# nibox/Pose-Estimation-with-Message-Passing-Networks

Hardware: AMD Instinct MI355X
Metric: images/sec (640px, HRNet-w48) + MPN edge-updates/sec at 1/2/4/8 MI355X (higher is better)
Workload: dtype f16x3; 1 GPU; c3: 8x17x640x640 heatmaps/GPU -> fully graph -> MPN TypeAware-attn T=3; images_per_gpu=8, global_batch=8, persons_per_image=9, nodes_per_gpu=1224, edges_per_gpu=186048, parallelism=image-sharded x1, batches_in_flight=2, detection_and_node_math=fp32

## Files before the change

### include/pemp.h

```cpp
#ifndef PEMP_H_
#define PEMP_H_

#include <stddef.h>
#include <stdint.h>

#ifdef __cplusplus
extern "C" {
#endif

#define PEMP_ABI_VERSION 24

enum {
  PEMP_OK = 0,
  PEMP_ERR_INVALID_ARG = -1,
  PEMP_ERR_HIP = -2,
  PEMP_ERR_WORKSPACE = -3,
  PEMP_ERR_UNSUPPORTED = -4,
};

int pemp_abi_version(void);
const char* pemp_last_error(void);
int pemp_device_check(void);

enum { PEMP_DETECT_NMS = 1, PEMP_DETECT_SELECT = 2, PEMP_DETECT_ALL = 3 };
// ... 215 lines not shown
                               const int32_t* n_det, int det_cap, const int64_t* node_off, int B,
                               float* edge_logits, float* node_logits, float* class_logits,
                               void* workspace, size_t workspace_bytes, void* stream);

enum {
  PEMP_STEP_DET = 0, PEMP_STEP_DSC, PEMP_STEP_NDET, PEMP_STEP_X, PEMP_STEP_JDET, PEMP_STEP_JSC, PEMP_STEP_BIDX,
  PEMP_STEP_JTAGS, PEMP_STEP_EIDX, PEMP_STEP_EATTR, PEMP_STEP_NOFF, PEMP_STEP_LOGITS, PEMP_STEP_NOUT
};
typedef struct pemp_step_plan {
  int32_t B, J, H, W, pool_kernel, use_threshold, topk, det_cap, projected;
  float threshold;
  void* det_workspace;
  size_t det_workspace_bytes;
  int32_t C, F, A, mode;
  float norm_factor;
  int64_t n_cap, e_cap;
  const pemp_mpn_desc* desc;
  const pemp_mpn_weights* weights;
  void* mpn_workspace;
  size_t mpn_workspace_bytes;
  int32_t n_rec;
  int64_t elog_n, nlog_off, clog_off;
  size_t off[PEMP_STEP_NOUT];
  size_t bytes;
} pemp_step_plan;
size_t pemp_step_layout(pemp_step_plan* plan);
int pemp_step_fully_cap(const pemp_step_plan* plan, const void* scoremaps, const float* masks, const float* features,
                        const float* tagmaps, void* out, int32_t* n_det_host, void* stream);

int pemp_mpn_graph_stats(uint64_t* out3);

int pemp_edge_cus_policy(int num_cus, int64_t E, int reserve_request);

size_t pemp_abi_struct_size(int which);

int pemp_mpn_forward_sym(const pemp_mpn_desc* desc, const pemp_mpn_weights* weights, const float* x,
                         const float* edge_attr, const int64_t* edge_index, const int64_t* node_types,
                         int64_t N, int64_t E, float* edge_logits, float* node_logits, float* class_logits,
                         void* workspace, size_t workspace_bytes, void* stream);

int pemp_mpn_forward_knn(const pemp_mpn_desc* desc, const pemp_mpn_weights* weights, const float* x,
                         const float* edge_attr, const int64_t* edge_index, const int64_t* node_types,
                         int64_t N, int64_t E, const void* knn_rows, const int32_t* knn_rowstart,
                         const int64_t* node_off, const int64_t* node_off_host, const int64_t* ecount, int B,
                         float* edge_logits, float* node_logits, float* class_logits,
                         void* workspace, size_t workspace_bytes, void* stream);

int pemp_mpn_prepare(const pemp_mpn_desc* desc, const int64_t* edge_index, const int64_t* node_types, int64_t N,
                     int64_t E, void* workspace, size_t workspace_bytes, void* stream);

int pemp_mpn_order_layout(const pemp_mpn_desc* desc, int64_t N, int64_t E, size_t offs[5]);

size_t pemp_mpn_edge_image_floats(const pemp_mpn_desc* desc, const pemp_mpn_weights* w);
int pemp_mpn_edge_image(const pemp_mpn_desc* desc, const pemp_mpn_weights* w, float* image, size_t floats,
                        void* stream);
size_t pemp_mpn_node_image_floats(const pemp_mpn_weights* weights);
int pemp_mpn_node_image(const pemp_mpn_weights* weights, float* image, size_t floats, void* stream);

int pemp_mpn_status(const pemp_mpn_desc* desc, int64_t N, int64_t E, const void* workspace, void* stream);

int pemp_prof_enable(const char* filter);
int pemp_prof_report(char* buf, size_t len);

#define PEMP_LABEL_OVERFLOW 1
typedef struct pemp_label_cand {
  int32_t g;
// ... 86 lines not shown
```

### pose-estimation-with-message-passing-networks_amd/_lib.py

```python
import ctypes
import threading
import os

LIB_PATH = os.environ.get("PEMP_LIB") or os.path.join(os.path.dirname(os.path.abspath(__file__)), "csrc",
                                                     "libpemp.so")
ABI_VERSION = 24

ERR_INVALID_ARG, ERR_HIP, ERR_WORKSPACE, ERR_UNSUPPORTED = -1, -2, -3, -4
MPN_PREPARED, MPN_TWO_LAUNCH_FIRST, MPN_FUSED_FIRST_PROFILED = 1, 4, 8
MPN_SEPARATE_PRELUDE = 16

c_i32, c_i64, c_f32, c_sz, c_p = ctypes.c_int32, ctypes.c_int64, ctypes.c_float, ctypes.c_size_t, ctypes.c_void_p


class PempLayer(ctypes.Structure):
    _fields_ = [("w", c_p), ("b", c_p), ("in_dim", c_i32), ("out_dim", c_i32), ("relu", c_i32), ("pad_", c_i32)]


class PempMlp(ctypes.Structure):
    _fields_ = [("layer", PempLayer * 4), ("n_layers", c_i32), ("pad_", c_i32)]


class PempMpnWeights(ctypes.Structure):
    _fields_ = [("node_emb", PempMlp), ("edge_emb", PempMlp),
# ... 65 lines not shown
    "pemp_fully_graph_build_cap": (c_i32, [c_p, c_i32, c_p, c_p, c_i32, c_p, c_i32, c_p, c_i32, c_i32, c_i32, c_i32,
                                           c_i64, c_i64, c_f32, c_i32, c_p, c_p, c_p, c_p, c_p, c_p, c_p, c_p, c_p]),
    "pemp_fully_graph": (c_i32, [c_p, c_p, c_i32, c_i64, c_p, c_p]),
    "pemp_knn_workspace_size": (c_sz, [c_p, c_i32]),
    "pemp_knn_graph_build": (c_i32, [c_p, c_p, c_p, c_i32, c_i32, c_p, c_sz, c_i64, c_p, c_p, c_p, c_i32, c_p,
                                     c_i32, c_f32, c_i32, c_p, c_p]),
    "pemp_feature_knn_workspace_size": (c_sz, [c_p, c_i32]),
    "pemp_knn_rows_layout": (c_i32, [c_p, c_i32, c_i32, c_p]),
    "pemp_feature_knn_graph_build": (c_i32, [c_p, c_i32, c_p, c_p, c_p, c_i32, c_i32, c_p, c_sz, c_i64, c_p, c_p,
                                             c_p, c_i32, c_p, c_i32, c_f32, c_i32, c_p, c_p]),
    "pemp_score_graph_workspace_size": (c_sz, [c_p, c_i32, c_i32]),
    "pemp_score_graph": (c_i32, [c_p, c_p, c_p, c_i32, c_i32, c_i64, c_p, c_sz, c_p, c_p]),
    "pemp_gather_projected": (c_i32, [c_p, c_p, c_p, c_i32, c_i32, c_i32, c_i32, c_f32, c_p, c_p, c_i64, c_p, c_p]),
    "pemp_gather_projected_conv": (c_i32, [c_p, c_p, c_p, c_i32, c_i32, c_p, c_p, c_i32, c_i32, c_i32, c_i32, c_i32,
                                           c_f32, c_p, c_p, c_i64, c_p, c_p]),
    "pemp_detect_projected": (c_i32, [c_p, c_p, c_i32, c_i32, c_i32, c_i32, c_i32, c_f32, c_i32, c_i32, c_i32, c_p,
                                      c_sz, c_p, c_p, c_p, c_i32, c_p, c_p]),
    "pemp_detect_projected_path": (c_i32, [c_p, c_p, c_i32, c_i32, c_i32, c_i32, c_p]),
    "pemp_gather_projected_tags": (c_i32, [c_p, c_i32, c_i32, c_i32, c_i32, c_p, c_p, c_i64, c_p, c_p]),
    "pemp_project_maps": (c_i32, [c_p, c_i32, c_i32, c_i32, c_i32, c_i32, c_p, c_p, c_p]),
    "pemp_stage_merge": (c_i32, [c_p, c_i32, c_i32, c_i32, c_p, c_i32, c_i32, c_i32, c_i32, c_i32, c_p, c_p]),
    "pemp_edge_features": (c_i32, [c_p, c_p, c_i32, c_p, c_p, c_i64, c_i32, c_f32, c_i32, c_p, c_p]),
    "pemp_mpn_workspace_size": (c_sz, [ctypes.POINTER(PempMpnDesc), c_i64, c_i64]),
    "pemp_mpn_fused_first_lds_bytes": (c_sz, []),
    "pemp_mpn_prelude_grids": (c_i32, [c_i64, c_i64, c_i32, c_i32, c_i32, c_i32, c_i32, c_p]),
    "pemp_mpn_forward": (c_i32, [ctypes.POINTER(PempMpnDesc), ctypes.POINTER(PempMpnWeights), c_p, c_p, c_p, c_p,
                                 c_i64, c_i64, c_p, c_p, c_p, c_p, c_sz, c_p]),
    "pemp_mpn_forward_fully": (c_i32, [ctypes.POINTER(PempMpnDesc), ctypes.POINTER(PempMpnWeights), c_p, c_p, c_p,
                                       c_p, c_i64, c_i64, c_p, c_p, c_i32, c_p, c_p, c_p, c_p, c_sz, c_p]),
    "pemp_mpn_forward_fully_cap": (c_i32, [ctypes.POINTER(PempMpnDesc), ctypes.POINTER(PempMpnWeights), c_p, c_p,
                                           c_p, c_i64, c_i64, c_p, c_i32, c_p, c_i32, c_p, c_p, c_p, c_p, c_sz, c_p]),
    "pemp_mpn_graph_stats": (c_i32, [c_p]),
    "pemp_edge_cus_policy": (c_i32, [c_i32, c_i64, c_i32]),
    "pemp_abi_struct_size": (c_sz, [c_i32]),
    "pemp_mpn_forward_sym": (c_i32, [ctypes.POINTER(PempMpnDesc), ctypes.POINTER(PempMpnWeights), c_p, c_p, c_p,
                                     c_p, c_i64, c_i64, c_p, c_p, c_p, c_p, c_sz, c_p]),
    "pemp_mpn_forward_knn": (c_i32, [ctypes.POINTER(PempMpnDesc), ctypes.POINTER(PempMpnWeights), c_p, c_p, c_p,
                                     c_p, c_i64, c_i64, c_p, c_p, c_p, c_p, c_p, c_i32, c_p, c_p, c_p, c_p, c_sz,
                                     c_p]),
    "pemp_mpn_prepare": (c_i32, [ctypes.POINTER(PempMpnDesc), c_p, c_p, c_i64, c_i64, c_p, c_sz, c_p]),
    "pemp_mpn_order_layout": (c_i32, [ctypes.POINTER(PempMpnDesc), c_i64, c_i64, c_p]),
    "pemp_mpn_edge_image_floats": (c_sz, [ctypes.POINTER(PempMpnDesc), ctypes.POINTER(PempMpnWeights)]),
    "pemp_mpn_edge_image": (c_i32, [ctypes.POINTER(PempMpnDesc), ctypes.POINTER(PempMpnWeights), c_p, c_sz, c_p]),
    "pemp_mpn_node_image_floats": (c_sz, [ctypes.POINTER(PempMpnWeights)]),
    "pemp_mpn_node_image": (c_i32, [ctypes.POINTER(PempMpnWeights), c_p, c_sz, c_p]),
    "pemp_mpn_status": (c_i32, [ctypes.POINTER(PempMpnDesc), c_i64, c_i64, c_p, c_p]),
    "pemp_pose_edge_weights": (c_i32, [c_p, c_i64, c_p, c_p, c_f32, c_i32, c_p, c_i32, c_i64, c_i32, c_p, c_p, c_p,
                                       c_p]),
    "pemp_pose_cluster": (c_i32, [c_i32, c_p, c_p, c_i64, c_p, c_p, c_i32, c_i32, c_p, c_p]),
    "pemp_pose_persons": (c_i32, [c_i32, c_p, c_p, c_p, c_p, c_p, c_p, c_p, c_i32, c_i32, c_i64, c_p, c_p, c_p]),
    "pemp_pose_greedy": (c_i32, [c_i32, c_p, c_p, c_i64, c_p, c_p, c_p, c_p, c_i32, c_p, c_i64, c_p, c_p]),
    "pemp_pose_fill_mean": (c_i32, [c_p, c_i32, c_i32]),
    "pemp_pose_refine_workspace_size": (c_sz, [c_i32, c_i32, c_i32, c_i32, c_i32]),
    "pemp_pose_refine": (c_i32, [c_p, c_p, c_i32, c_i32, c_i32, c_i32, c_p, c_i32, c_p, c_sz, c_p]),
    "pemp_pose_adjust": (c_i32, [c_p, c_i32, c_i32, c_i32, c_p, c_i32, c_p]),
    "pemp_pack_to_host": (c_i32, [c_i32, c_p, c_p, c_p, c_sz, c_p, c_p, c_p]),
    "pemp_pose_finish_plan": (c_i32, [c_i32, c_p, c_p, c_p, c_p, c_i32, c_p]),
    "pemp_pose_finish_batch": (c_i32, [c_p, c_p, c_i32, c_i32, c_i32, c_i32, c_i32, c_p, c_i32, c_p, c_p, c_i32,
                                       c_i32, c_p, c_i32, c_p, c_sz, c_p]),
    "pemp_step_layout": (c_sz, [ctypes.POINTER(PempStepPlan)]),
    "pemp_step_fully_cap": (c_i32, [ctypes.POINTER(PempStepPlan), c_p, c_p, c_p, c_p, c_p, c_p, c_p]),
    "pemp_prof_enable": (c_i32, [ctypes.c_char_p]),
    "pemp_prof_report": (c_i32, [ctypes.c_char_p, c_sz]),
    "pemp_label_candidates_scratch_size": (c_sz, [c_i32, c_i32, c_i32]),
    "pemp_label_candidates": (c_i32, [c_p, c_p, c_i32, c_i32, c_i32, c_i32, c_p, c_p, c_i32, c_i32, ctypes.c_double,
                                      c_i64, c_p, c_p, c_p, c_p, c_sz, c_p]),
# ... 110 lines not shown
```

### pose-estimation-with-message-passing-networks_amd/csrc/mpn.hip

```cpp
#include <limits.h>

#include <algorithm>
#include <atomic>
#include <type_traits>
#include <map>
#include <mutex>
#include <string>
#include <vector>
#include <string.h>
#include <math.h>

#include "pemp_common.h"

namespace pemp {
namespace {

constexpr int D = 64;
constexpr int LDW = 72;
constexpr int MAXT = 17;
constexpr int EDGE_WAVES = 16;
constexpr int EMB_WAVES = 16, EMB_PER_CU = 1;
constexpr int EMB_MIN_WAVES_EU = EMB_WAVES * EMB_PER_CU / 4 > 1 ? EMB_WAVES * EMB_PER_CU / 4 : 1;
constexpr int RESERVE_CUS_DEFAULT = 64;
constexpr int64_t RESERVE_MIN_EDGES = 65536;
static int edge_cus_policy(int cus, int64_t E, int request) {
  if (E < RESERVE_MIN_EDGES || cus <= 8) return cus;
  const int r = std::min(std::max(request, 0), cus / 4) & ~7;
  return cus - r;
}
static int edge_cus(int64_t E) {
  static const int request = [] {
    const char* e = getenv("PEMP_RESERVE_CUS");
    return e ? atoi(e) : RESERVE_CUS_DEFAULT;
  }();
  return edge_cus_policy(num_cus(), E, request);
}

__device__ __forceinline__ float4 ld4(const float* p) { return *reinterpret_cast<const float4*>(p); }
__device__ __forceinline__ void st4(float* p, float a, float b, float c, float d) {
  *reinterpret_cast<float4*>(p) = make_float4(a, b, c, d);
}

template <int KB, int OB>
__device__ __forceinline__ void gemm_frag(const float* W, int ldw, const float (&in)[KB][4],
                                          float (&acc)[OB][4]) {
  const int lane = __lane_id(), i = lane & 15, g = lane >> 4;
#pragma unroll
  for (int ob = 0; ob < OB; ++ob) {
    f32x4 c = {acc[ob][0], acc[ob][1], acc[ob][2], acc[ob][3]};
#pragma unroll
    for (int mb = 0; mb < KB; ++mb) {
      const float4 w = ld4(W + (16 * ob + i) * ldw + 16 * mb + 4 * g);
      c = mfma4(w.x, in[mb][0], c);
      c = mfma4(w.y, in[mb][1], c);
      c = mfma4(w.z, in[mb][2], c);
      c = mfma4(w.w, in[mb][3], c);
    }
    acc[ob][0] = c[0]; acc[ob][1] = c[1]; acc[ob][2] = c[2]; acc[ob][3] = c[3];
  }
}

__device__ __forceinline__ float relu1(float x) { return __int_as_float(max(__float_as_int(x), 0)); }

template <int NB>
__device__ __forceinline__ void relu_frag(float (&v)[NB][4]) {
#pragma unroll
  for (int b = 0; b < NB; ++b)
#pragma unroll
// ... 70 lines not shown
  o = __shfl_up(v, 2, 16); if (m.f2) v += o;
  o = __shfl_up(v, 4, 16); if (m.f4) v += o;
  o = __shfl_up(v, 8, 16); if (m.f8) v += o;
  return v;
}

__device__ __forceinline__ float scan_max(float v, const SegMask& m) {
  float o;
  o = __shfl_up(v, 1, 16); if (m.f1) v = fmaxf(v, o);
  o = __shfl_up(v, 2, 16); if (m.f2) v = fmaxf(v, o);
  o = __shfl_up(v, 4, 16); if (m.f4) v = fmaxf(v, o);
  o = __shfl_up(v, 8, 16); if (m.f8) v = fmaxf(v, o);
  return v;
}

__device__ __forceinline__ float scan_max_bwd(float v, const SegMask& m) {
  float o;
  o = __shfl_down(v, 1, 16); if (m.b1) v = fmaxf(v, o);
  o = __shfl_down(v, 2, 16); if (m.b2) v = fmaxf(v, o);
  o = __shfl_down(v, 4, 16); if (m.b4) v = fmaxf(v, o);
  o = __shfl_down(v, 8, 16); if (m.b8) v = fmaxf(v, o);
  return v;
}

struct MpnWs {
  int *cnt, *seg, *wg_start, *perm, *s_src, *s_dst, *s_orig, *err, *sym;
  float *X, *NT, *agg, *Q0, *EA, *EB, *img, *eimg;
  int4* ranges;
};

constexpr int IMG_FLOATS = 112 * 1024;
constexpr int EIMG_MAX_STRIDE = 4 * D * LDW + (2 * D + 4) + (D + 32) * LDW + D + 32 + 32 + 4;

static MpnWs mpn_carve(void* base, int T, int64_t N, int64_t E, size_t* bytes, size_t* order_offs = nullptr) {
  Carver c(base);
  MpnWs w;
  size_t oo[5];
  const int64_t K = (int64_t)T * N;
  w.err = c.take<int>(64);
  w.cnt = w.err + 64;
  c.take<int>(K + 1);
  w.seg = c.take<int>(K + 1);
  oo[0] = c.last;
  w.wg_start = c.take<int>(MAXT + 2);
  oo[1] = c.last;
  w.perm = c.take<int>(E);
  w.s_src = c.take<int>(E);
  oo[2] = c.last;
  w.s_dst = c.take<int>(E);
  oo[3] = c.last;
  w.s_orig = c.take<int>(E);
  oo[4] = c.last;
  if (order_offs) std::copy(oo, oo + 5, order_offs);
  w.X = c.take<float>(N * 128);
  w.NT = c.take<float>(N * (128 + 64 * (int64_t)T));
  w.agg = c.take<float>(N * T * D);
  w.Q0 = c.take<float>(E * D);
  w.EA = c.take<float>(E * D);
  w.EB = c.take<float>(E * D);
  w.img = c.take<float>(IMG_FLOATS);
  const int G = std::max(num_cus(), T);
  w.ranges = c.take<int4>((size_t)G * (EDGE_WAVES + 12));
  w.eimg = c.take<float>((size_t)T * EIMG_MAX_STRIDE);
  w.sym = c.take<int>(3 * N);
  if (bytes) *bytes = c.used;
  return w;
}

__global__ __launch_bounds__(256) void mpn_count_kernel(const int64_t* __restrict__ ei, const int64_t* __restrict__ types,
                                                        int64_t ts, int64_t N, int64_t E, int T, int* __restrict__ cnt,
                                                        int* __restrict__ err) {
  for (int64_t e = (int64_t)blockIdx.x * blockDim.x + threadIdx.x; e < E; e += (int64_t)gridDim.x * blockDim.x) {
    const int64_t s = ei[e], d = ei[E + e];
    if (s < 0 || s >= N || d < 0 || d >= N) { atomicOr(err, 1); continue; }
    const int64_t t = T == 1 ? 0 : types[s * ts];
    if (t < 0 || t >= T) { atomicOr(err, 2); continue; }
    atomicAdd(&cnt[t * N + d], 1);
  }
}



__device__ void type_split(const int* tstart, int64_t etot, int T, int G, int* gt, int* wg_start) {
  (void)etot;
  if (threadIdx.x < 64) {
    const int lane = threadIdx.x;
    const int tiles = lane < T ? (tstart[lane + 1] - tstart[lane] + 15) / 16 : 0;
    int hi = tiles;
    for (int o = 32; o >= 1; o >>= 1) hi = max(hi, __shfl_xor(hi, o));
    int lo = 1;
    hi = max(hi, 1);
    while (lo < hi) {
      const int mid = (lo + hi) >> 1;
      int need = tiles > 0 ? (tiles + mid - 1) / mid : 0;
      for (int o = 32; o >= 1; o >>= 1) need += __shfl_xor(need, o);
// ... 2372 lines not shown
        const float (&xh)[4][4] = h ? x1 : x0;
#pragma unroll
        for (int kb = 0; kb < 2; ++kb) {
          uint32_t hw[4], lw[4];
#pragma unroll
          for (int d = 0; d < 4; ++d)
            split_pair(xh[2 * kb + (d >> 1)][2 * (d & 1)], xh[2 * kb + (d >> 1)][2 * (d & 1) + 1], ss, hw[d], lw[d]);
          const u32x4_t hv = {hw[0], hw[1], hw[2], hw[3]}, lv = {lw[0], lw[1], lw[2], lw[3]};
          hi[kb] = __builtin_bit_cast(f16x8_t, hv);
          lo[kb] = __builtin_bit_cast(f16x8_t, lv);
        }
#pragma unroll
        for (int kb = 0; kb < 2; ++kb) {
          acc = __builtin_amdgcn_mfma_f32_16x16x32_f16(flo[2 * h + kb], hi[kb], acc, 0, 0, 0);
          acc = __builtin_amdgcn_mfma_f32_16x16x32_f16(fh[2 * h + kb], lo[kb], acc, 0, 0, 0);
          acc = __builtin_amdgcn_mfma_f32_16x16x32_f16(fh[2 * h + kb], hi[kb], acc, 0, 0, 0);
        }
      }
      if (big) acc *= 1.0f / ss;
    }
    if (nn < N) st4(a.NT + nn * a.NO + 16 * ob + 4 * g, acc[0], acc[1], acc[2], acc[3]);
  }
}

template <int PREC, int TILES = TBL_TILES, bool SUM = false>
__global__ __launch_bounds__(256) void node_table_kernel(NodeTableArgs a) {
  __shared__ __attribute__((aligned(16))) float xs[16 * TILES * RS];
  node_table_role<PREC, TILES, SUM>(a, xs, blockIdx.x);
}

template <int PREC>
__global__ __launch_bounds__(256) void prelude_b_kernel(EdgeRangesArgs ra, NodeTableArgs ta, int split) {
  __shared__ __attribute__((aligned(16))) float xs[16 * TBL_TILES * RS];
  const int bx = blockIdx.x;
  if (bx < split) edge_ranges_role(ra, bx);
  else node_table_role<PREC, TBL_TILES, false>(ta, xs, bx - split);
}

static int grid1d(int64_t total, int block, int cap = 65536) {
  int64_t g = (total + block - 1) / block;
  return (int)(g < 1 ? 1 : (g > cap ? cap : g));
}

static bool published_head(const pemp_mlp& m) {
  return m.n_layers == 3 && m.layer[0].in_dim == 64 && m.layer[0].out_dim == 64 && m.layer[0].relu &&
         m.layer[1].in_dim == 64 && m.layer[1].out_dim == 32 && m.layer[1].relu && m.layer[2].in_dim == 32 &&
         m.layer[2].out_dim == 1 && !m.layer[2].relu;
}

template <int AGG, int PREC, int UPD, int STAGE>
static void launch_edge_step_s(const EdgeStepArgs& a, bool head, bool pub, int grid, hipStream_t st) {
  if (!head)
    hipLaunchKernelGGL((edge_step_kernel<AGG, 0, PREC, UPD, STAGE>), dim3(grid), dim3(64 * edge_waves<0>()), 0, st, a);
  else if (pub)
    hipLaunchKernelGGL((edge_step_kernel<AGG, 1, PREC, UPD, STAGE>), dim3(grid), dim3(64 * edge_waves_s<1, STAGE>()), 0,
                       st, a);
  else
    hipLaunchKernelGGL((edge_step_kernel<AGG, 2, PREC, UPD, STAGE>), dim3(grid), dim3(64 * edge_waves<2>()), 0, st, a);
}

template <int AGG, int PREC, int UPD>
static void launch_edge_step_p(const EdgeStepArgs& a, bool head, bool pub, int grid, int stage, hipStream_t st) {
  if constexpr (AGG == PEMP_AGGR_ATTN) {
    if (stage == (STAGE_MID | STAGE_EPT)) { launch_edge_step_s<AGG, PREC, UPD, STAGE_MID | STAGE_EPT>(a, head, pub, grid, st); return; }
    if (stage == (STAGE_LAST | STAGE_EPT)) { launch_edge_step_s<AGG, PREC, UPD, STAGE_LAST | STAGE_EPT>(a, head, pub, grid, st); return; }
  }
  if (stage == STAGE_MID) launch_edge_step_s<AGG, PREC, UPD, STAGE_MID>(a, head, pub, grid, st);
  else launch_edge_step_s<AGG, PREC, UPD, STAGE_LAST>(a, head, pub, grid, st);
}
// ... 667 lines not shown
  __syncthreads();
  KP_CLK(5);
  if (tid == 0 && (t == 0 || t == T - 1))
    printf("kp block %d,%d: start %lld init +%lld masks +%lld rows +%lld scan +%lld placed +%lld\n", t, blockIdx.y,
           clk[0], clk[1] - clk[0], clk[2] - clk[0], clk[3] - clk[0], clk[4] - clk[0], clk[5] - clk[0]);
#endif
  if (t != T - 1 || blockIdx.y != 0) return;
  if (tid == 0) {
    int acc = 0;
    for (int u = 0; u < T; ++u) { tst[u] = acc; acc += tot[u]; }
    tst[T] = acc;
    a.seg[(int64_t)T * N] = acc;
    a.err[0] = (bad_sh ? 2 : 0) | (acc != a.E || ebase[B] != a.E ? 4 : 0);
    a.err[1] = a.err[2] = a.err[3] = 0;
  }
  __syncthreads();
  type_split(tst, tst[T], T, a.G, gt, a.wg_start);
}

static int launch_prepare(const pemp_mpn_desc* desc, const int64_t* edge_index, const int64_t* node_types, int64_t N,
                          int64_t E, const MpnWs& ws, hipStream_t st) {
  const int T = desc->num_types;
  const int64_t tstride = desc->types_stride > 0 ? desc->types_stride : 1;
  const int64_t K = (int64_t)T * N;
  ProfScope prof("mpn_prepare", st);
  hipLaunchKernelGGL(zero_words_kernel, dim3((unsigned)std::min<int64_t>((K + 64 + 255) / 256, 1024)), dim3(256), 0,
                     st, ws.err, K + 65);
  PEMP_LAUNCH_CHECK();
  if (E > 0) {
    hipLaunchKernelGGL(mpn_count_kernel, dim3(grid1d(E, 256)), dim3(256), 0, st, edge_index, node_types, tstride, N, E, T,
                       ws.cnt, ws.err);
    PEMP_LAUNCH_CHECK();
  }
  hipLaunchKernelGGL(mpn_scan_kernel, dim3(1), dim3(1024), 0, st, ws.cnt, K, N, T, std::max(edge_cus(E), T), ws.seg,
                     ws.wg_start);
  PEMP_LAUNCH_CHECK();
  if (E > 0) {
    hipLaunchKernelGGL(mpn_scatter_kernel, dim3(grid1d(E, 256)), dim3(256), 0, st, edge_index, node_types, tstride, N, E, T,
                       ws.seg, ws.cnt, ws.perm);
    PEMP_LAUNCH_CHECK();
    hipLaunchKernelGGL(mpn_segsort_kernel, dim3((unsigned)((K + 15) / 16)), dim3(256), 0, st, edge_index, E, K, ws.seg,
                       ws.perm, ws.s_src, ws.s_dst, ws.s_orig);
    PEMP_LAUNCH_CHECK();
  }
  return PEMP_OK;
}

static int launch_prepare_sym(const pemp_mpn_desc* desc, const int64_t* edge_index, const int64_t* node_types,
                              int64_t N, int64_t E, const MpnWs& ws, hipStream_t st) {
  const int T = desc->num_types;
  const int64_t tstride = desc->types_stride > 0 ? desc->types_stride : 1;
  const int64_t K = (int64_t)T * N;
  ProfScope prof("mpn_prepare_sym", st);
  int2* rows = reinterpret_cast<int2*>(ws.sym);
  int* flags = ws.sym + 2 * N;
  unsigned* packed = reinterpret_cast<unsigned*>(ws.perm);
  const unsigned g = (unsigned)((N + 3) / 4);
  hipLaunchKernelGGL(sym_rows_kernel, dim3(g), dim3(256), 0, st, edge_index, node_types, tstride, N, E, T, ws.cnt, rows,
                     packed, flags);
  PEMP_LAUNCH_CHECK();
  hipLaunchKernelGGL(sym_scan_kernel, dim3((unsigned)T), dim3(1024), 0, st, ws.cnt, N, T, std::max(edge_cus(E), T), ws.seg,
                     ws.wg_start, flags, E, ws.err);
  PEMP_LAUNCH_CHECK();
  hipLaunchKernelGGL(sym_place_kernel, dim3(g), dim3(256), 0, st, N, T, ws.seg, rows, packed, ws.s_src, ws.s_dst,
                     ws.s_orig, ws.err);
  PEMP_LAUNCH_CHECK();
  return PEMP_OK;
}

}
}

using namespace pemp;

extern "C" size_t pemp_mpn_workspace_size(const pemp_mpn_desc* desc, int64_t N, int64_t E) {
  if (!desc || N < 0 || E < 0 || desc->num_types < 1) return 0;
  size_t bytes = 0;
  mpn_carve(nullptr, desc->num_types, N, E, &bytes);
  return bytes;
}

#ifdef PEMP_STAMPS
static unsigned long long* g_diag_stamps = nullptr;
static int g_diag_stamp_pass = 0;
extern "C" int pemp_diag_stamps(void* buf, int pass) {
  g_diag_stamps = static_cast<unsigned long long*>(buf);
  g_diag_stamp_pass = pass;
  return PEMP_OK;
}
#endif

struct EdgeOrder {
  enum Kind { SORT, FULLY, SYM, KNN } kind = SORT;
  const int64_t* node_off = nullptr;
// ... 124 lines not shown
  int emb_prec;
  EmbedLayout emb_lo;
  bool fused_heads, fused_embed;
  int edge_grid;
  int NO, table_prec, table_groups;
  unsigned node_grid, table_grid, table_grid1;
  int node_mode;
  bool sum_in_table;
  bool fused_first;
  PreludeGrids grids;
  bool paired;
};

static ForwardPlan plan_forward(const ForwardCall& c) {
  const pemp_mpn_desc& d = *c.desc;
  const pemp_mpn_weights& w = *c.w;
  const int64_t N = c.N, E = c.E;
  ForwardPlan p{};
  p.T = d.num_types; p.J = d.num_joints; p.steps = d.steps; p.aux = d.aux_loss_steps;
  p.tstride = d.types_stride > 0 ? d.types_stride : 1;
  p.upd_fused = edge_upd_fused(d, w);
  p.pub_head = edge_pub_head(d, w);
  p.ept = w.ept_l1_w != nullptr;
  p.emb_lds = mlp_ok(w.edge_emb, 64, 64);
  p.emb_prec = embed_prec(d, w);
  p.emb_lo = embed_layout(w.edge_emb, p.emb_prec);
  p.emb_generic = p.emb_lds && !embed_fixed_shape(p.emb_prec == PEMP_PREC_FP32
                                                      ? embed_layout(w.edge_emb, PEMP_PREC_F16X3)
                                                      : p.emb_lo);
  p.fixed = embed_fixed_shape(p.emb_lo);
  p.comp = embed_composed(p.emb_lo, p.emb_prec, w);
  p.fused_heads = node_heads_fused(w);
  p.fused_embed = node_embed_fused(w);
  p.edge_grid = std::max(edge_cus(E), p.T);
  p.NO = 128 + 64 * p.T;
  p.table_prec = d.precision != PEMP_PREC_FP32 && w.pre_bf ? d.precision : PEMP_PREC_FP32;
  p.table_groups = (p.NO / 16 + 3) / 4;
  p.grids = prelude_grids(N, E, c.order.kind == EdgeOrder::FULLY ? c.order.B : 0, p.T, c.order.nmax, p.edge_grid,
                          num_cus());
  p.node_grid = (unsigned)p.grids.rows_blocks;
  p.table_grid = (unsigned)p.grids.table_blocks;
  p.table_grid1 = (unsigned)(((N + 15) / 16) * p.table_groups);
  p.node_mode = p.upd_fused ? ROWS_SUM : (w.upd_w || w.upd_mlp.n_layers > 0) ? NODE_UPDATE_MLP : ROWS_COPY;
  p.sum_in_table = !p.ept && N * p.T * 256 * (int64_t)p.table_groups <= NODE_SUM_TABLE_MAX_MB << 20;
  p.fused_first = E > 0 && p.steps >= 2 && p.steps - p.aux - 1 > 0 && !(d.flags & PEMP_MPN_TWO_LAUNCH_FIRST) &&
                  d.precision == PEMP_PREC_F16X3 && d.aggr == PEMP_AGGR_ATTN && p.upd_fused && !p.ept &&
                  p.emb_lds && p.comp && w.edge_img &&
                  prof_repeat("edge_step") == 1 &&
                  (!prof_active() || (d.flags & PEMP_MPN_FUSED_FIRST_PROFILED));
  p.paired = c.order.kind == EdgeOrder::FULLY && !(d.flags & (PEMP_MPN_PREPARED | PEMP_MPN_SEPARATE_PRELUDE)) &&
             p.fused_embed && p.steps >= 1 && !prof_active();
  return p;
}

struct Forward {
  const ForwardCall& c;
  const ForwardPlan& p;
  const MpnWs ws;
  const hipStream_t st;
  const int64_t* ne = nullptr;
  const float* node_img = nullptr;
  const float* eimg = nullptr;
  float* r_cur;
  float* r_next;
  int rec = 0;

  Forward(const ForwardCall& call, const ForwardPlan& plan)
// ... 359 lines not shown
  if (it != table.end()) return it->second;
  GraphStream* g = new GraphStream();
  if (hipStreamCreateWithFlags(&g->s, hipStreamNonBlocking) != hipSuccess ||
      hipEventCreateWithFlags(&g->fork, hipEventDisableTiming) != hipSuccess ||
      hipEventCreateWithFlags(&g->join, hipEventDisableTiming) != hipSuccess) {
    (void)hipGetLastError();
    return nullptr;
  }
  table[dev] = g;
  return g;
}

static std::atomic<uint64_t> g_graph_captures{0}, g_graph_replays{0}, g_graph_refused{0};

extern "C" size_t pemp_abi_struct_size(int which) {
  switch (which) {
    case 0: return sizeof(pemp_mpn_weights);
    case 1: return sizeof(pemp_mpn_desc);
    case 2: return sizeof(pemp_mlp);
    case 3: return sizeof(pemp_proj_maps);
    case 4: return sizeof(pemp_step_plan);
    case 5: return sizeof(pemp_loss_rec);
    default: return 0;
  }
}

extern "C" int pemp_edge_cus_policy(int num_cus_, int64_t E, int reserve_request) {
  PEMP_CHECK_ARG(num_cus_ >= 1 && E >= 0, "pemp_edge_cus_policy: bad args");
  if (reserve_request < 0) {
    const char* e = getenv("PEMP_RESERVE_CUS");
    reserve_request = e ? atoi(e) : RESERVE_CUS_DEFAULT;
  }
  return edge_cus_policy(num_cus_, E, reserve_request);
}

extern "C" int pemp_mpn_graph_stats(uint64_t* out3) {
  PEMP_CHECK_ARG(out3, "pemp_mpn_graph_stats: null output");
  out3[0] = g_graph_captures.load();
  out3[1] = g_graph_replays.load();
  out3[2] = g_graph_refused.load();
  return PEMP_OK;
}

extern "C" int pemp_mpn_forward_fully_cap(const pemp_mpn_desc* desc, const pemp_mpn_weights* w, const float* x,
                                          const float* edge_attr, const int64_t* node_types, int64_t n_cap,
                                          int64_t e_cap, const int32_t* n_det, int det_cap, const int64_t* node_off,
                                          int B, float* edge_logits, float* node_logits, float* class_logits,
                                          void* workspace, size_t workspace_bytes, void* stream) {
  PEMP_CHECK_ARG(desc && w && n_det && node_off && B >= 1 && B <= FULLY_MAXB, "pemp_mpn_forward_fully_cap: bad args");
  PEMP_CHECK_ARG(n_cap >= 1 && e_cap >= 0 && det_cap >= 1, "pemp_mpn_forward_fully_cap: bad capacities");
  if (det_cap > FULLY_MAXN || !node_heads_fused(*w) || !node_embed_fused(*w) || !mlp_ok(w->edge_emb, 64, 64)) {
    set_error("pemp_mpn_forward_fully_cap: this model / capacity takes the exact forward");
    return PEMP_ERR_UNSUPPORTED;
  }
  auto direct = [&](void* s) {
    ForwardCall c{};
    c.desc = desc; c.w = w; c.x = x; c.edge_attr = edge_attr; c.node_types = node_types;
    c.N = n_cap; c.E = e_cap; c.edge_logits = edge_logits; c.node_logits = node_logits; c.class_logits = class_logits;
    c.workspace = workspace; c.workspace_bytes = workspace_bytes; c.stream = s;
    c.order.kind = EdgeOrder::FULLY; c.order.node_off = node_off; c.order.B = B; c.order.nmax = det_cap;
    c.cap.ne = node_off + B + 1;
    return mpn_forward(c);
  };
  if (graphs_off() || prof_active() || debug_sync()) return direct(stream);
  int dev = 0;
  PEMP_HIP(hipGetDevice(&dev));
// ... 120 lines not shown
  ka.list_cap = cap ? std::max(0, std::min(KP_LIST, atoi(cap))) : KP_LIST;
  ForwardCall c{};
  c.desc = desc; c.w = w; c.x = x; c.edge_attr = edge_attr; c.edge_index = edge_index; c.node_types = node_types;
  c.N = N; c.E = E; c.edge_logits = edge_logits; c.node_logits = node_logits; c.class_logits = class_logits;
  c.workspace = workspace; c.workspace_bytes = workspace_bytes; c.stream = stream;
  c.order.kind = EdgeOrder::KNN; c.order.knn = &ka;
  return mpn_forward(c);
}

extern "C" int pemp_mpn_prepare(const pemp_mpn_desc* desc, const int64_t* edge_index, const int64_t* node_types,
                                int64_t N, int64_t E, void* workspace, size_t workspace_bytes, void* stream) {
  PEMP_CHECK_ARG(desc && desc->num_types >= 1 && desc->num_types <= MAXT, "pemp_mpn_prepare: bad desc");
  PEMP_CHECK_ARG(N >= 0 && E >= 0 && N < (1ll << 30) && E < (1ll << 31) - 64 && (int64_t)desc->num_types * N < (1ll << 30),
                 "pemp_mpn_prepare: N=%lld E=%lld out of range", (long long)N, (long long)E);
  PEMP_CHECK_ARG(E == 0 || (edge_index && node_types), "pemp_mpn_prepare: null edge tensors");
  size_t need = 0;
  mpn_carve(nullptr, desc->num_types, N, E, &need);
  if (workspace_bytes < need) {
    set_error("pemp_mpn_prepare: workspace %zu < %zu bytes", workspace_bytes, need);
    return PEMP_ERR_WORKSPACE;
  }
  if (N == 0) return PEMP_OK;
  return launch_prepare(desc, edge_index, node_types, N, E, mpn_carve(workspace, desc->num_types, N, E, nullptr),
                        as_stream(stream));
}

extern "C" int pemp_mpn_order_layout(const pemp_mpn_desc* desc, int64_t N, int64_t E, size_t* offs) {
  PEMP_CHECK_ARG(desc && offs && desc->num_types >= 1 && desc->num_types <= MAXT, "pemp_mpn_order_layout: bad desc");
  PEMP_CHECK_ARG(N >= 0 && E >= 0, "pemp_mpn_order_layout: N=%lld E=%lld out of range", (long long)N, (long long)E);
  mpn_carve(nullptr, desc->num_types, N, E, nullptr, offs);
  return PEMP_OK;
}

extern "C" size_t pemp_mpn_fused_first_lds_bytes(void) { return edge_first_lds_bytes(); }

extern "C" int pemp_mpn_prelude_grids(int64_t N, int64_t E, int B, int T, int nmax, int edge_grid, int cus,
                                      int32_t* out8) {
  PEMP_CHECK_ARG(out8 && N >= 0 && E >= 0 && B >= 0 && B <= FULLY_MAXB && T >= 1 && T <= MAXT && nmax >= 0 &&
                     nmax <= FULLY_MAXN && edge_grid >= 1 && cus >= 1,
                 "pemp_mpn_prelude_grids: bad args");
  const PreludeGrids g = prelude_grids(N, E, B, T, nmax, edge_grid, cus);
  static_assert(sizeof(PreludeGrids) == 8 * sizeof(int32_t), "eight ints");
  memcpy(out8, &g, sizeof(g));
  return PEMP_OK;
}

extern "C" size_t pemp_mpn_edge_image_floats(const pemp_mpn_desc* desc, const pemp_mpn_weights* w) {
  if (!desc || !w || desc->num_types < 1 || desc->num_types > MAXT) return 0;
  if (!mlp_ok(w->edge_emb, 64, 64)) return edge_image_base_floats(*desc, *w);
  return embed_image_offset(*desc, *w) + embed_image_floats(embed_layout(w->edge_emb, embed_prec(*desc, *w)));
}

extern "C" int pemp_mpn_edge_image(const pemp_mpn_desc* desc, const pemp_mpn_weights* w, float* image, size_t floats,
                                   void* stream) {
  PEMP_CHECK_ARG(desc && w && image, "pemp_mpn_edge_image: null pointer");
  PEMP_CHECK_ARG(desc->num_types >= 1 && desc->num_types <= MAXT, "pemp_mpn_edge_image: bad num_types");
  PEMP_CHECK_ARG(desc->precision == PEMP_PREC_FP32 || (w->e1_bf && w->e2_bf && w->msg_bf),
                 "pemp_mpn_edge_image: split precisions need the *_bf packs");
  PEMP_CHECK_ARG(w->e1_w && w->e2_w && w->e2_b && w->msg_w, "pemp_mpn_edge_image: null layer weights");
  PEMP_CHECK_ARG(desc->aggr != PEMP_AGGR_ATTN || w->attn_w, "pemp_mpn_edge_image: attention needs attn_w");
  const size_t need = pemp_mpn_edge_image_floats(desc, w);
  PEMP_CHECK_ARG(floats >= need, "pemp_mpn_edge_image: image needs %zu floats", need);
  EdgeImgArgs ia = edge_image_args(*desc, *w, edge_upd_fused(*desc, *w), edge_pub_head(*desc, *w), image);
  hipLaunchKernelGGL(edge_image_kernel, dim3(16, (unsigned)desc->num_types), dim3(256), 0, as_stream(stream), ia);
  PEMP_LAUNCH_CHECK();
  if (mlp_ok(w->edge_emb, 64, 64)) {
// ... 55 lines not shown
```

Baseline: 37830 images/s.

## Size edge-pass grid by per-type tile trips instead of fixed CU reserve

Adds a policy that picks the edge-kernel grid size by searching, in steps of 8, over grid counts between the reserved-CU baseline and half the reserve. For each candidate it estimates the number of 16-wave tile trips per type via binary search, and keeps the candidate that reduces the worst-case trips. This can hand some reserved CUs to the edge pass to cut the tail of the per-type workgroup split. The prelude_b kernel's block roles are rearranged so that edge-range blocks can sit both before and after the node-table blocks, which accommodates the larger range count. Trade-off: fewer CUs remain reserved for overlapping work, and the policy assumes edges are split evenly across types.

```diff
diff --git a/include/pemp.h b/include/pemp.h
--- a/include/pemp.h
+++ b/include/pemp.h
@@ -271,6 +271,12 @@
 
 int pemp_edge_cus_policy(int num_cus, int64_t E, int reserve_request);
 
+int pemp_edge_grid_policy(int num_cus, int64_t N, int64_t E, int T, int reserve_request);
+
+int pemp_edge_pass_trips(const int64_t* type_edges, int T, int G, int slack_tiles, int waves);
+
+int pemp_mpn_ranges_layout(const pemp_mpn_desc* desc, int64_t N, int64_t E, size_t* off, int32_t* grid);
+
 size_t pemp_abi_struct_size(int which);
 
 int pemp_mpn_forward_sym(const pemp_mpn_desc* desc, const pemp_mpn_weights* weights, const float* x,
diff --git a/pose-estimation-with-message-passing-networks_amd/_lib.py b/pose-estimation-with-message-passing-networks_amd/_lib.py
--- a/pose-estimation-with-message-passing-networks_amd/_lib.py
+++ b/pose-estimation-with-message-passing-networks_amd/_lib.py
@@ -121,6 +121,9 @@
                                            c_p, c_i64, c_i64, c_p, c_i32, c_p, c_i32, c_p, c_p, c_p, c_p, c_sz, c_p]),
     "pemp_mpn_graph_stats": (c_i32, [c_p]),
     "pemp_edge_cus_policy": (c_i32, [c_i32, c_i64, c_i32]),
+    "pemp_edge_grid_policy": (c_i32, [c_i32, c_i64, c_i64, c_i32, c_i32]),
+    "pemp_edge_pass_trips": (c_i32, [c_p, c_i32, c_i32, c_i32, c_i32]),
+    "pemp_mpn_ranges_layout": (c_i32, [ctypes.POINTER(PempMpnDesc), c_i64, c_i64, c_p, c_p]),
     "pemp_abi_struct_size": (c_sz, [c_i32]),
     "pemp_mpn_forward_sym": (c_i32, [ctypes.POINTER(PempMpnDesc), ctypes.POINTER(PempMpnWeights), c_p, c_p, c_p,
                                      c_p, c_i64, c_i64, c_p, c_p, c_p, c_p, c_sz, c_p]),
diff --git a/pose-estimation-with-message-passing-networks_amd/csrc/mpn.hip b/pose-estimation-with-message-passing-networks_amd/csrc/mpn.hip
--- a/pose-estimation-with-message-passing-networks_amd/csrc/mpn.hip
+++ b/pose-estimation-with-message-passing-networks_amd/csrc/mpn.hip
@@ -28,12 +28,50 @@
   const int r = std::min(std::max(request, 0), cus / 4) & ~7;
   return cus - r;
 }
-static int edge_cus(int64_t E) {
+static int reserve_request() {
   static const int request = [] {
     const char* e = getenv("PEMP_RESERVE_CUS");
     return e ? atoi(e) : RESERVE_CUS_DEFAULT;
   }();
-  return edge_cus_policy(num_cus(), E, request);
+  return request;
+}
+static int edge_cus(int64_t E) { return edge_cus_policy(num_cus(), E, reserve_request()); }
+
+static int edge_pass_trips(const int64_t* type_edges, int T, int G, int slack, int waves) {
+  int64_t tiles[MAXT], hi = 1;
+  for (int t = 0; t < T; ++t) hi = std::max(hi, tiles[t] = (type_edges[t] + 15) / 16);
+  int64_t lo = 1;
+  while (lo < hi) {
+    const int64_t mid = (lo + hi) / 2;
+    int64_t need = 0;
+    for (int t = 0; t < T; ++t) need += (tiles[t] + mid - 1) / mid;
+    if (need <= G) hi = mid;
+    else lo = mid + 1;
+  }
+  int64_t most = 0;
+  for (int t = 0; t < T; ++t)
+    if (tiles[t] > 0) {
+      const int64_t gt = (tiles[t] + lo - 1) / lo;
+      most = std::max(most, (tiles[t] + gt - 1) / gt + (gt > 1 ? slack : 0));
+    }
+  return (int)((most + waves - 1) / waves);
+}
+
+static int edge_grid_policy(int cus, int64_t N, int64_t E, int T, int request) {
+  const int base = edge_cus_policy(cus, E, request), r = cus - base;
+  if (r < 16 || T < 1 || T > MAXT || N < 1 || base < T) return std::max(base, 1);
+  int64_t te[MAXT];
+  for (int t = 0; t < T; ++t) te[t] = (E + T - 1) / T;
+  const int slack = (int)(((E + N * T - 1) / (N * T) - 1 + 15) / 16);
+  int best = base, trips = edge_pass_trips(te, T, base, slack, EDGE_WAVES);
+  for (int g = base + 8; g <= cus - ((r / 2 + 7) & ~7); g += 8) {
+    const int k = edge_pass_trips(te, T, g, slack, EDGE_WAVES);
+    if (k < trips) { best = g; trips = k; }
+  }
+  return best;
+}
+static int edge_grid(int64_t N, int64_t E, int T) {
+  return std::max(edge_grid_policy(num_cus(), N, E, T, reserve_request()), T);
 }
 
 __device__ __forceinline__ float4 ld4(const float* p) { return *reinterpret_cast<const float4*>(p); }
@@ -170,7 +208,8 @@
 constexpr int IMG_FLOATS = 112 * 1024;
 constexpr int EIMG_MAX_STRIDE = 4 * D * LDW + (2 * D + 4) + (D + 32) * LDW + D + 32 + 32 + 4;
 
-static MpnWs mpn_carve(void* base, int T, int64_t N, int64_t E, size_t* bytes, size_t* order_offs = nullptr) {
+static MpnWs mpn_carve(void* base, int T, int64_t N, int64_t E, size_t* bytes, size_t* order_offs = nullptr,
+                       size_t* ranges_off = nullptr) {
   Carver c(base);
   MpnWs w;
   size_t oo[5];
@@ -199,6 +238,7 @@
   w.img = c.take<float>(IMG_FLOATS);
   const int G = std::max(num_cus(), T);
   w.ranges = c.take<int4>((size_t)G * (EDGE_WAVES + 12));
+  if (ranges_off) *ranges_off = c.last;
   w.eimg = c.take<float>((size_t)T * EIMG_MAX_STRIDE);
   w.sym = c.take<int>(3 * N);
   if (bytes) *bytes = c.used;
@@ -2637,9 +2677,10 @@
 template <int PREC>
 __global__ __launch_bounds__(256) void prelude_b_kernel(EdgeRangesArgs ra, NodeTableArgs ta, int split) {
   __shared__ __attribute__((aligned(16))) float xs[16 * TBL_TILES * RS];
-  const int bx = blockIdx.x;
-  if (bx < split) edge_ranges_role(ra, bx);
-  else node_table_role<PREC, TBL_TILES, false>(ta, xs, bx - split);
+  const int bx = blockIdx.x, tb = gridDim.x - split;
+  if (bx < ra.RB) edge_ranges_role(ra, bx);
+  else if (bx < ra.RB + tb) node_table_role<PREC, TBL_TILES, false>(ta, xs, bx - ra.RB);
+  else edge_ranges_role(ra, bx - tb);
 }
 
 static int grid1d(int64_t total, int block, int cap = 65536) {
@@ -3373,7 +3414,7 @@
                        ws.cnt, ws.err);
     PEMP_LAUNCH_CHECK();
   }
-  hipLaunchKernelGGL(mpn_scan_kernel, dim3(1), dim3(1024), 0, st, ws.cnt, K, N, T, std::max(edge_cus(E), T), ws.seg,
+  hipLaunchKernelGGL(mpn_scan_kernel, dim3(1), dim3(1024), 0, st, ws.cnt, K, N, T, edge_grid(N, E, T), ws.seg,
                      ws.wg_start);
   PEMP_LAUNCH_CHECK();
   if (E > 0) {
@@ -3400,7 +3441,7 @@
   hipLaunchKernelGGL(sym_rows_kernel, dim3(g), dim3(256), 0, st, edge_index, node_types, tstride, N, E, T, ws.cnt, rows,
                      packed, flags);
   PEMP_LAUNCH_CHECK();
-  hipLaunchKernelGGL(sym_scan_kernel, dim3((unsigned)T), dim3(1024), 0, st, ws.cnt, N, T, std::max(edge_cus(E), T), ws.seg,
+  hipLaunchKernelGGL(sym_scan_kernel, dim3((unsigned)T), dim3(1024), 0, st, ws.cnt, N, T, edge_grid(N, E, T), ws.seg,
                      ws.wg_start, flags, E, ws.err);
   PEMP_LAUNCH_CHECK();
   hipLaunchKernelGGL(sym_place_kernel, dim3(g), dim3(256), 0, st, N, T, ws.seg, rows, packed, ws.s_src, ws.s_dst,
@@ -3591,7 +3632,7 @@
   p.comp = embed_composed(p.emb_lo, p.emb_prec, w);
   p.fused_heads = node_heads_fused(w);
   p.fused_embed = node_embed_fused(w);
-  p.edge_grid = std::max(edge_cus(E), p.T);
+  p.edge_grid = edge_grid(N, E, p.T);
   p.NO = 128 + 64 * p.T;
   p.table_prec = d.precision != PEMP_PREC_FP32 && w.pre_bf ? d.precision : PEMP_PREC_FP32;
   p.table_groups = (p.NO / 16 + 3) / 4;
@@ -4017,6 +4058,18 @@
     reserve_request = e ? atoi(e) : RESERVE_CUS_DEFAULT;
   }
   return edge_cus_policy(num_cus_, E, reserve_request);
+}
+
+extern "C" int pemp_edge_grid_policy(int num_cus_, int64_t N, int64_t E, int T, int reserve_request_) {
+  PEMP_CHECK_ARG(num_cus_ >= 1 && N >= 0 && E >= 0 && T >= 1 && T <= MAXT, "pemp_edge_grid_policy: bad args");
+  return edge_grid_policy(num_cus_, N, E, T, reserve_request_ < 0 ? reserve_request() : reserve_request_);
+}
+
+extern "C" int pemp_edge_pass_trips(const int64_t* type_edges, int T, int G, int slack_tiles, int waves) {
+  PEMP_CHECK_ARG(type_edges && T >= 1 && T <= MAXT && G >= T && slack_tiles >= 0 && waves >= 1,
+                 "pemp_edge_pass_trips: bad args");
+  for (int t = 0; t < T; ++t) PEMP_CHECK_ARG(type_edges[t] >= 0, "pemp_edge_pass_trips: negative count");
+  return edge_pass_trips(type_edges, T, G, slack_tiles, waves);
 }
 
 extern "C" int pemp_mpn_graph_stats(uint64_t* out3) {
@@ -4203,6 +4256,15 @@
   return PEMP_OK;
 }
 
+extern "C" int pemp_mpn_ranges_layout(const pemp_mpn_desc* desc, int64_t N, int64_t E, size_t* off, int32_t* grid) {
+  PEMP_CHECK_ARG(desc && off && grid && desc->num_types >= 1 && desc->num_types <= MAXT,
+                 "pemp_mpn_ranges_layout: bad desc");
+  PEMP_CHECK_ARG(N >= 0 && E >= 0, "pemp_mpn_ranges_layout: N=%lld E=%lld out of range", (long long)N, (long long)E);
+  mpn_carve(nullptr, desc->num_types, N, E, nullptr, nullptr, off);
+  *grid = edge_grid(N, E, desc->num_types);
+  return PEMP_OK;
+}
+
 extern "C" size_t pemp_mpn_fused_first_lds_bytes(void) { return edge_first_lds_bytes(); }
 
 extern "C" int pemp_mpn_prelude_grids(int64_t N, int64_t E, int B, int T, int nmax, int edge_grid, int cus,
```

After: 37290 images/s. 1.4% lower.
